# Lqm26/BMCNet-ESR

Hardware: AMD Instinct MI355X
Metric: LR-voxel-frames/sec x4 SR train step, NFS-shaped 180x240 (BASELINE configs[1] / [2]), f32 (higher is better)
Workload: dtype f32; 1 GPU; BMCNet(scale=4, n_c=128, n_b=5) x4 SR train step, NFS-shaped 180x240 (BASELINE configs[1] / [2]) -> 720x960, bs=4/GPU, arithmetic fp32 (native fp32 MFMA; 3x3 convolutions through Winograd F(4x4,3x3) / F(2x2,3x3) transforms in fp32), SEQL=9 SEQN=2 (8 windows BPTT), event scatter + fwd + MSE + bwd + Adam(amsgrad); global_batch=4, parallelism=dp1, rccl_ranks=1, rccl_initialised_before_headline_run=False

## Files before the change

### bmcnet-esr_amd/bmc_hip/lib.py

```python
from __future__ import annotations

import ctypes as C
import os

import torch

_HERE = os.path.dirname(os.path.abspath(__file__))
LIB_PATH = os.environ.get("BMC_HIP_LIB") or os.path.join(os.path.dirname(_HERE), "csrc", "libbmc_hip.so")

if not os.path.exists(LIB_PATH):
    raise ImportError(
        f"{LIB_PATH} not found: build the HIP extension first "
        "(python -c 'import __graft_entry__ as g; g.build()' or make -C bmcnet-esr_amd/csrc). "
        "The BMCNet MI355X path has no CPU fallback.")

_lib = C.CDLL(LIB_PATH)

MAX_SRC = 6
c_fp = C.c_void_p


class Src(C.Structure):
    _fields_ = [("ptr", C.c_void_p), ("batch_stride", C.c_longlong), ("pix_stride", C.c_int), ("nch", C.c_int),
                ("batch_shift", C.c_int), ("batch_mod", C.c_int)]


class ConvArgs(C.Structure):
    _fields_ = [("nsrc", C.c_int), ("src", Src * MAX_SRC), ("wpacked", C.c_void_p), ("bias", C.c_void_p),
                ("w_group_stride", C.c_longlong), ("bias_group_stride", C.c_int), ("batch_per_group", C.c_int),
                ("out", C.c_void_p), ("out_batch_stride", C.c_longlong), ("out_pix_stride", C.c_int),
                ("B", C.c_int), ("H", C.c_int), ("W", C.c_int), ("Cout", C.c_int), ("Coutpad", C.c_int),
                ("taps", C.c_int), ("relu", C.c_int), ("residual", Src), ("mask", Src), ("accumulate", C.c_int),
                ("math", C.c_int)]


class PgemmArgs(C.Structure):
    _fields_ = [("a", Src), ("nsrc", C.c_int), ("src", Src * MAX_SRC), ("B", C.c_int), ("H", C.c_int), ("W", C.c_int),
                ("taps", C.c_int), ("batch_per_group", C.c_int), ("slabs", C.c_void_p), ("nsplit", C.c_int),
                ("zeros", C.c_void_p), ("bias_slabs", C.c_void_p), ("math", C.c_int), ("tap_groups", C.c_int)]


class ChainFwdArgs(C.Structure):
    _fields_ = [("s0", Src), ("s1", Src), ("wstream", C.c_void_p), ("bias_f", C.c_void_p), ("bias_c", C.c_void_p),
                ("gamma", C.c_void_p), ("beta", C.c_void_p), ("eps", C.c_float), ("yhat", C.c_void_p), ("rstd", C.c_void_p),
                ("centre", C.c_void_p), ("B", C.c_int), ("C", C.c_int), ("H", C.c_int), ("W", C.c_int)]


class ChainBwdArgs(C.Structure):
    _fields_ = [("dcentre", Src), ("wstream", C.c_void_p), ("gamma", C.c_void_p), ("yhat", C.c_void_p), ("rstd", C.c_void_p),
                ("dz", C.c_void_p), ("ds1", C.c_void_p), ("ds0", C.c_void_p), ("ds0_add", Src), ("n", C.c_int), ("C", C.c_int),
                ("H", C.c_int), ("W", C.c_int)]


class MmTerm(C.Structure):
    _fields_ = [("a", C.c_void_p), ("a_sb", C.c_longlong), ("a_sg", C.c_longlong), ("a_si", C.c_int), ("a_sk", C.c_int),
                ("b", C.c_void_p), ("b_sb", C.c_longlong), ("b_sg", C.c_longlong), ("b_sk", C.c_int), ("b_sj", C.c_int),
                ("w", C.c_void_p), ("w_sb", C.c_longlong), ("w_sg", C.c_longlong), ("w_sk", C.c_int)]


class SmallMmArgs(C.Structure):
    _fields_ = [("nterms", C.c_int), ("t", MmTerm * 2), ("nbatch", C.c_int), ("batch_per_group", C.c_int),
                ("M", C.c_int), ("N", C.c_int), ("K", C.c_int), ("alpha", C.c_float),
                ("u", C.c_void_p), ("u_sb", C.c_longlong), ("u_sg", C.c_longlong),
                ("v", C.c_void_p), ("v_sb", C.c_longlong), ("v_sg", C.c_longlong),
                ("c", C.c_void_p), ("c_sb", C.c_longlong), ("c_sg", C.c_longlong), ("c_si", C.c_int), ("c_sj", C.c_int),
                ("vec_out", C.c_void_p), ("vo_sb", C.c_longlong), ("vo_sg", C.c_longlong), ("accumulate", C.c_int)]


def _sig(name, argtypes, restype=C.c_int):
    fn = getattr(_lib, name)
    fn.argtypes = argtypes
    fn.restype = restype
    return fn


_ll, _i, _f, _p = C.c_longlong, C.c_int, C.c_float, C.c_void_p

bmc_version = _sig("bmc_version", [])
bmc_last_error = _sig("bmc_last_error", [], C.c_char_p)
_events = _sig("bmc_events_to_channels", [_p, _p, _p, _p, _i, _i, _i, _p, _i, _p])
_voxel = _sig("bmc_events_to_voxel", [_p, _p, _p, _p, _p, _ll, _i, _i, _i, _i, _p, _i, _p, _p])
_stack_pol = _sig("bmc_events_to_stack_polarity", [_p, _p, _p, _p, _ll, _p, _p, _i, _i, _i, _p, _p, _i, _p])
_mask = _sig("bmc_events_to_mask", [_p, _p, _p, _ll, _i, _i, _p, _p, _i, _p])
_stack = _sig("bmc_events_to_stack", [_p, _p, _p, _p, _ll, _p, _p, _i, _i, _i, _p, _p, _i, _p])
_enc_raw = _sig("bmc_encode_raw_events", [_p, _p, _p, _p, _p, _i, _i, _i, _p, _p])
_events_ws = _sig("bmc_events_binned_ws_bytes", [_ll, _i, _i, _i], C.c_longlong)
_events_binned = _sig("bmc_events_to_channels_binned", [_p, _p, _p, _p, _ll, _i, _i, _i, _p, _i, _p, _ll, _p])
_enc_raw_binned = _sig("bmc_encode_raw_events_binned", [_p, _p, _p, _p, _p, _ll, _i, _i, _i, _p, _p, _ll, _p])
_ev_torch_ws = _sig("bmc_events_torch_ws_ints", [_ll, _i, _i], C.c_longlong)
_ev_img_torch = _sig("bmc_events_to_image_torch", [_p, _p, _p, _ll, _i, _i, _i, _i, _i, _p, _p, _p])
_ev_vox_torch = _sig("bmc_events_to_voxel_torch", [_p, _p, _p, _p, _ll, _i, _i, _i, _p, _p, _p])
_pack_w = _sig("bmc_pack_weight", [_p, _p, _i, _i, _i, _i, _i, _i, _p, _p])
_pack_wt = _sig("bmc_pack_weight_t", [_p, _p, _i, _i, _i, _i, _i, _i, _i, _i, _p, _p])
_pack_wino = _sig("bmc_pack_weight_wino", [_p, _p, _i, _i, _i, _i, _i, _i, _i, _i, _p, _p])
_pack_wino4 = _sig("bmc_pack_weight_wino4", [_p, _p, _i, _i, _i, _i, _i, _i, _i, _i, _p, _p])
_ww_nsplit = _sig("bmc_wgrad_wino_nsplit", [_i, _i, _i])
_stream_low = _sig("bmc_stream_create_low_priority", [C.POINTER(C.c_void_p)])
_small_mm = _sig("bmc_small_mm", [C.POINTER(SmallMmArgs), _p])
_ww = _sig("bmc_wgrad_wino", [C.POINTER(Src), C.POINTER(Src), _i, _i, _i, _i, _p, _p, _p])
_ww_red = _sig("bmc_wgrad_wino_reduce", [_p, _i, _p, _i, _i, _i, _p, _p, _p])
_ww_multi = _sig("bmc_wgrad_wino_multi", [C.POINTER(Src), C.POINTER(Src), C.POINTER(C.c_int), _i, _i, _i, _i, _p, _p, _p])
_ptr_table = _sig("bmc_ptr_table", [C.POINTER(C.c_ulonglong), _i, _p, _p])
_wino_rows = _sig("bmc_conv_wino_rows", [_i, _i, _i, _i, _i])
_ww4_nsplit = _sig("bmc_wgrad_wino4_nsplit", [_i, _i, _i])
_ww4 = _sig("bmc_wgrad_wino4", [C.POINTER(Src), C.POINTER(Src), _i, _i, _i, _i, _p, _p, _p])
_ww4_red = _sig("bmc_wgrad_wino4_reduce", [_p, _i, _p, _i, _i, _i, _p, _p, _p])
_split_w = _sig("bmc_split_weight", [_p, _p, _ll, _i, _i, _p])
_conv = _sig("bmc_conv", [C.POINTER(ConvArgs), _p])
_pgemm = _sig("bmc_pgemm", [C.POINTER(PgemmArgs), _p])
_red_w = _sig("bmc_pgemm_reduce_weight", [_p, _i, _i, _i, _i, _i, _p, _i, _p, _i, _p, _p, _p])
_red_wg = _sig("bmc_pgemm_reduce_weight_groups", [_p, _i, _i, _i, _i, _i, _p, _i, _p, _i, _p, _p, _p])
_red_p = _sig("bmc_pgemm_reduce_plain", [_p, _i, _i, _i, _i, _f, _p, _p])
_colsum = _sig("bmc_colsum", [_p, _ll, _i, _i, _p, _p, _i, _p])
_relu_bwd = _sig("bmc_relu_bwd", [_p, _p, _p, _ll, _p])
_ln_fwd = _sig("bmc_layernorm_fwd", [_p, _p, _p, _ll, _i, _f, _p, _p, _p])
_ln_bwd = _sig("bmc_layernorm_bwd", [_p, _p, _p, _p, _ll, _i, _p, _p, _p, _p, _i, _p])
_sm_fwd = _sig("bmc_softmax_fwd", [_p, _ll, _i, _p, _p])
_sm_bwd = _sig("bmc_softmax_bwd", [_p, _p, _ll, _i, _f, _p, _p])
_pack_in = _sig("bmc_pack_inputs", [_p, _ll, _ll, _ll, _ll, _ll, _i, _i, _i, _i, _p, _p, _p])
_unshuffle = _sig("bmc_unshuffle_to_nhwc", [_p, _i, _i, _i, _i, _i, _p, _i, _p])
_shuffle = _sig("bmc_shuffle_to_hr", [_p, _i, _i, _i, _i, _i, _p, _ll, _ll, _ll, _ll, _p, _i, _p])
_head_mse_fwd = _sig("bmc_head_mse_fwd", [_p, _i, _i, _i, _i, _i, _p, _ll, _ll, _ll, _ll, _p, _ll, _p, _p, _p, _p])
_head_mse_bwd = _sig("bmc_head_mse_bwd", [_p, _p, _p, _ll, _p, _i, _i, _i, _i, _i, _p, _p])
_group_sum = _sig("bmc_group_sum", [_p, _i, _ll, _p, _p])
_bicubic_fwd = _sig("bmc_bicubic_resize_fwd", [_p, _ll, _i, _i, _i, _i, _p, _p])
_bicubic_bwd = _sig("bmc_bicubic_resize_bwd", [_p, _ll, _i, _i, _i, _i, _p, _p])
_chain_fwd = _sig("bmc_chain_fwd", [C.POINTER(ChainFwdArgs), _p])
_chain_bwd = _sig("bmc_chain_bwd", [C.POINTER(ChainBwdArgs), _p])
_chain_affine = _sig("bmc_chain_affine_grads", [_p, _p, _p, _p, _p, _i, _p, _p, _p, _p, _i, _p])
_slot_stage = _sig("bmc_slot_stage", [_p, _i, _i, _i, _i, _p, _p, _i, _p, _i, _ll, _p, _ll, _p])
_slot_commit = _sig("bmc_slot_commit", [_p, _i, C.POINTER(C.c_void_p), _i, _ll, _p, _i, _p, _p, _ll, _p])
_slot_metrics = _sig("bmc_slot_metrics", [_p, _i, _p, _i, _i, _i, _i, _i, _i, _i, _p])
_slot_encode = _sig("bmc_slot_encode", [_p, _i, _i, _i, _i, _i, _i, _p, _p, _p])
_slot_emit = _sig("bmc_slot_emit", [_p, _p, _i, _p, _i, _i, _i, _i, _p, _p])
_slot_emit_timed = _sig("bmc_slot_emit_timed", [_p, _p, _i, _p, _i, _i, _i, _i, _p, _p, _p, _ll, _p])
_slot_emit_clocked = _sig("bmc_slot_emit_clocked", [_p, _p, _p, _i, _p, _i, _i, _i, _i, _p, _p, _p, _ll, _p])
_slot_emit_timed_ws = _sig("bmc_slot_emit_timed_scratch_bytes", [_i, _i, _ll], C.c_longlong)
_slot_hot_update = _sig("bmc_slot_hot_update", [_p, _p, _i, _i, _i, _i, _i, _i, _p, _p, _p, _p])
_slot_encode_filtered = _sig("bmc_slot_encode_filtered", [_p, _p, _p, _i, _i, _i, _i, _i, _i, _p, _p, _p])
_hot_pixel_mask = _sig("bmc_hot_pixel_mask", [_p, _i, _i, _i, _i, _f, _p, _p, _p])
_slot_render = _sig("bmc_slot_render", [_p, _p, _i, _i, _i, _i, _i, _p, _p])

EXPORTS = ["bmc_version", "bmc_last_error", "bmc_events_to_channels", "bmc_events_to_voxel", "bmc_events_to_stack", "bmc_encode_raw_events", "bmc_pack_weight", "bmc_pack_weight_t", "bmc_split_weight", "bmc_conv",
           "bmc_pgemm", "bmc_pgemm_reduce_weight", "bmc_pgemm_reduce_plain", "bmc_colsum", "bmc_relu_bwd",
           "bmc_layernorm_fwd", "bmc_layernorm_bwd", "bmc_softmax_fwd", "bmc_softmax_bwd", "bmc_pack_inputs",
           "bmc_unshuffle_to_nhwc", "bmc_shuffle_to_hr", "bmc_bicubic_resize_fwd", "bmc_bicubic_resize_bwd",
           "bmc_chain_fwd", "bmc_chain_bwd", "bmc_chain_affine_grads", "bmc_group_sum",
           "bmc_head_mse_fwd", "bmc_head_mse_bwd", "bmc_events_to_stack_polarity", "bmc_events_to_mask",
           "bmc_pgemm_reduce_weight_groups", "bmc_events_binned_ws_bytes", "bmc_events_to_channels_binned",
           "bmc_encode_raw_events_binned", "bmc_pack_weight_wino", "bmc_pack_weight_wino4", "bmc_wgrad_wino_nsplit", "bmc_wgrad_wino",
           "bmc_wgrad_wino_reduce", "bmc_events_torch_ws_ints", "bmc_events_to_image_torch",
           "bmc_events_to_voxel_torch", "bmc_stream_create_low_priority", "bmc_small_mm",
           "bmc_wgrad_wino4_nsplit", "bmc_wgrad_wino4", "bmc_wgrad_wino4_reduce", "bmc_wgrad_wino_multi", "bmc_ptr_table",
           "bmc_conv_wino_rows", "bmc_slot_stage", "bmc_slot_commit", "bmc_slot_metrics", "bmc_slot_encode", "bmc_slot_emit",
           "bmc_slot_emit_timed", "bmc_slot_emit_timed_scratch_bytes", "bmc_slot_emit_clocked", "bmc_slot_hot_update",
           "bmc_slot_encode_filtered", "bmc_hot_pixel_mask", "bmc_slot_render"]


def check(rc, what):
    if rc != 0:
        raise RuntimeError(f"{what} failed (rc={rc}): {bmc_last_error().decode()}")


def call(fn, what, *args):
    check(fn(*args), what)


def has_symbol(name: str) -> bool:
    return hasattr(_lib, name)
```

### bmcnet-esr_amd/csrc/pgemm.hip

```cpp
#include "bmc_common.h"
#include "pgemm_k.h"
#include "dma_ring.h"

namespace {


template <int TAPS, int TG = TAPS, bool TAB = false>
__global__ __launch_bounds__(512, 2) void pgemm_dma_kernel(const PgemmK a) {
    constexpr int HWD = PT_W + 2, HHT = PT_H + 2;
    constexpr int NHALO = TAPS == 9 ? HWD * HHT : PT;
    constexpr int XCH = TAPS == 9 ? 64 : 128;
    constexpr int NT = TAPS == 9 ? 1 : 2;
    constexpr int XSH = TAPS == 9 ? 4 : 5;
    constexpr int BUF = 2048 * 4;
    __shared__ __attribute__((aligned(16))) float lds[4 * BUF];
    __shared__ SrcDev tab[BMC_MAX_SRC];
    const int tid = threadIdx.x, lane = tid & 63;
    BMC_LOAD_SRC_TABLE(tab, a, tid);
    __syncthreads();
    const int wave = __builtin_amdgcn_readfirstlane(tid >> 6);
    const int li = lane & 31, lh = lane >> 5;
    const int mw = wave & 3, nw = wave >> 2;

    int bid = blockIdx.x;
    const int split = bid % a.nsplit; bid /= a.nsplit;
    const int tg = TG == TAPS ? 0 : bid % (TAPS / TG);
    if (TG != TAPS) bid /= TAPS / TG;
    const int nb = bid % a.n_nblk; bid /= a.n_nblk;
    const int mb = bid % a.n_mblk;
    const int g = bid / a.n_mblk;
    const int m0 = mb * 128, n0 = nb * XCH;
    const bool wave_active = m0 + 32 * mw < a.Mpad;
    const int HWp = a.H * a.W;

    f32x16 acc[TG * NT];
#pragma unroll
    for (int t = 0; t < TG * NT; ++t)
#pragma unroll
        for (int r = 0; r < 16; ++r) acc[t][r] = 0.f;

    const int ntiles = a.batch_per_group * a.tiles_per_img;
    int xsi = 0, xch0 = n0;
#pragma unroll
    for (int si = 1; si < BMC_MAX_SRC; ++si)
        if (xsi == si - 1 && xch0 >= tab[si - 1].nch && si < a.nsrc) { xch0 -= tab[si - 1].nch; xsi = si; }
    const SrcDev xs = tab[xsi];
    const bool x_one_src = xch0 + XCH <= xs.nch;
    int a_off[4], x_off[4], a_yx[4], x_yx[4];
#pragma unroll
    for (int i = 0; i < 4; ++i) {
        const int e = i * 512 + tid, p = e >> 5, c4 = (e & 31) * 4;
        a_yx[i] = TAPS == 9 ? ((p >> 4) << 16) | (p & 15) : p;
        a_off[i] = ((TAPS == 9 ? (p >> 4) * a.W + (p & 15) : p) * a.a.pix_stride + m0 + c4) * 4;
        const int hp = e >> XSH, xc4 = (e & ((1 << XSH) - 1)) * 4;
        const int hy = TAPS == 9 ? hp / HWD : 0, hx = TAPS == 9 ? hp - hy * HWD : hp;
        x_yx[i] = TAPS == 9 ? (hy << 16) | hx : hp;
        x_off[i] = ((TAPS == 9 ? (hp < NHALO ? hy * a.W + hx : 0) : hp) * xs.pix_stride + xch0 + xc4) * 4;
    }
    const bool all_ch = m0 + 128 <= a.M && n0 + XCH <= a.N && x_one_src &&
                        (long long)a.H * a.W * (a.a.pix_stride > xs.pix_stride ? a.a.pix_stride : xs.pix_stride) < (1ll << 28);
    const int step_img = a.nsplit / a.tiles_per_img, step_rem = a.nsplit - step_img * a.tiles_per_img;
    const int step_ty = TAPS == 9 ? step_rem / a.tiles_x : 0, step_tx = TAPS == 9 ? step_rem - step_ty * a.tiles_x : step_rem;
    int nx_bb = split / a.tiles_per_img, nx_ty, nx_tx;
    {
        const int tin = split - nx_bb * a.tiles_per_img;
        nx_ty = TAPS == 9 ? tin / a.tiles_x : 0; nx_tx = TAPS == 9 ? tin - nx_ty * a.tiles_x : tin;
    }
    auto dma = [&](const void* sbase, unsigned voff, float* ldst) { dma16(sbase, voff, lds_addr(ldst)); };
    auto issue = [&](int tile, int buf) {
        const int b = g * a.batch_per_group + nx_bb;
        int y0 = 0, x0 = 0, p0 = 0;
        if (TAPS == 9) { y0 = nx_ty * PT_H; x0 = nx_tx * PT_W; }
        else p0 = nx_tx * PT;
        nx_bb += step_img; nx_ty += step_ty; nx_tx += step_tx;
        if (TAPS == 9) {
            if (nx_tx >= a.tiles_x) { nx_tx -= a.tiles_x; ++nx_ty; }
            if (nx_ty >= a.tiles_y) { nx_ty -= a.tiles_y; ++nx_bb; }
        } else if (nx_tx >= a.tiles_per_img) { nx_tx -= a.tiles_per_img; ++nx_bb; }
        const float* ab = src_bp<TAB>(a.a, b);
        const bool interior = TAPS == 9 ? (y0 >= 1 && x0 >= 1 && y0 + PT_H + 1 <= a.H && x0 + PT_W + 1 <= a.W) : (p0 + PT <= HWp);
        if (interior && all_ch) {
            const float* const abt = ab + (TAPS == 9 ? (long long)y0 * a.W + x0 : (long long)p0) * a.a.pix_stride;
            const float* const xbt = src_bp<TAB>(xs, b) +
                                     (TAPS == 9 ? (long long)(y0 - 1) * a.W + (x0 - 1) : (long long)p0) * xs.pix_stride;
#pragma unroll
            for (int i = 0; i < 4; ++i) dma(abt, (unsigned)a_off[i], lds + buf * BUF + (i * 512 + wave * 64) * 4);
#pragma unroll
            for (int i = 0; i < 4; ++i) dma(xbt, (unsigned)x_off[i], lds + (2 + buf) * BUF + (i * 512 + wave * 64) * 4);
            return;
        }
#pragma unroll
        for (int i = 0; i < 4; ++i) {
            const int e = i * 512 + tid, p = e >> 5, c4 = (e & 31) * 4;
            long long pix;
            bool ok;
            if (TAPS == 9) {
                const int y = y0 + (p >> 4), x = x0 + (p & 15);
                ok = y < a.H && x < a.W;
                pix = (long long)y * a.W + x;
            } else {
                pix = p0 + p;
                ok = pix < HWp;
            }
            const float* src = a.zeros;
            if (ok && m0 + c4 < a.M) src = ab + pix * a.a.pix_stride + m0 + c4;
            dma16v(src, lds_addr(lds + buf * BUF + (i * 512 + wave * 64) * 4));
        }
#pragma unroll
        for (int i = 0; i < 4; ++i) {
            const int e = i * 512 + tid, hp = e >> XSH, c4 = (e & ((1 << XSH) - 1)) * 4;
            long long pix;
            bool ok;
            if (TAPS == 9) {
                const int hy = hp / HWD, hx = hp - hy * HWD;
                const int y = y0 - 1 + hy, x = x0 - 1 + hx;
                ok = hp < NHALO && y >= 0 && y < a.H && x >= 0 && x < a.W;
                pix = (long long)y * a.W + x;
            } else {
                pix = p0 + hp;
                ok = pix < HWp;
            }
            int ch = n0 + c4;
            const float* src = a.zeros;
            if (ok && ch < a.N) {
                int s_i = 0;
#pragma unroll
                for (int si = 1; si < BMC_MAX_SRC; ++si)
                    if (s_i == si - 1 && ch >= tab[si - 1].nch && si < a.nsrc) { ch -= tab[si - 1].nch; s_i = si; }
                const SrcDev S = tab[s_i];
                src = src_bp<TAB>(S, b) + pix * S.pix_stride + ch;
            }
            dma16v(src, lds_addr(lds + (2 + buf) * BUF + (i * 512 + wave * 64) * 4));
        }
    };

    if (split < ntiles) issue(split, 0);
    dma_wait<0>();
    __syncthreads();
    const bool do_bias = a.bias_slabs != nullptr && nb == 0 && tg == 0;
    float bsum = 0.f;
    int it = 0;
    for (int tile = split; tile < ntiles; tile += a.nsplit, ++it) {
        const int cur = it & 1;
        const int next = tile + a.nsplit;
        if (next < ntiles) issue(next, cur ^ 1);
        if (do_bias) {
            const float* const bp = lds + cur * BUF + (tid >> 7) * 16 * 128 + (tid & 127);
#pragma unroll
            for (int r = 0; r < 16; ++r) bsum += bp[r * 128];
        }
        if (wave_active) {
            const float* const ap = lds + cur * BUF + lh * 128 + 32 * mw + li;
            const float* const xp = lds + (2 + cur) * BUF + lh * XCH + 32 * NT * nw + li + (TG == TAPS ? 0 : tg * HWD * XCH);
            if constexpr (TAPS == 1) {
                constexpr int QB = 4, NBAT = PT / 2 / QB;
                float av[2][QB], xv[2][QB][NT];
                auto rd = [&](const int slot, const int q0) __attribute__((always_inline)) {
#pragma unroll
                    for (int j = 0; j < QB; ++j) {
                        av[slot][j] = ap[2 * (q0 + j) * 128];
#pragma unroll
                        for (int u = 0; u < NT; ++u) xv[slot][j][u] = xp[2 * (q0 + j) * XCH + 32 * u];
                    }
                };
                rd(0, 0);
#pragma unroll
                for (int qb = 0; qb < NBAT; ++qb) {
                    if (qb + 1 < NBAT) rd((qb + 1) & 1, (qb + 1) * QB);
                    __builtin_amdgcn_sched_barrier(0);
#pragma unroll
                    for (int j = 0; j < QB; ++j)
#pragma unroll
                        for (int u = 0; u < NT; ++u)
                            acc[u] = __builtin_amdgcn_mfma_f32_32x32x2f32(av[qb & 1][j], xv[qb & 1][j][u], acc[u], 0, 0, 0);
                    __builtin_amdgcn_sched_barrier(0);
                }
            } else
#pragma unroll
            for (int q = 0; q < PT / 2; ++q) {
                const float av = ap[2 * q * 128];
#pragma unroll
                for (int tap = 0; tap < TG; ++tap)
#pragma unroll
                    for (int u = 0; u < NT; ++u) {
                        int off;
                        if (TAPS == 9) off = (((q >> 3) + tap / 3) * HWD + 2 * (q & 7) + tap % 3) * XCH;
                        else off = 2 * q * XCH + 32 * u;
                        acc[tap * NT + u] = __builtin_amdgcn_mfma_f32_32x32x2f32(av, xp[off], acc[tap * NT + u], 0, 0, 0);
                    }
            }
        }
        dma_wait<0>();
        __syncthreads();
    }

    if (do_bias && m0 + (tid & 127) < a.Mpad)
        a.bias_slabs[(((long long)split * a.G + g) * 4 + (tid >> 7)) * a.Mpad + m0 + (tid & 127)] = bsum;
    if (wave_active) {
        float* const sl = a.slabs + (((long long)split * a.G + g) * TAPS + (TG == TAPS ? 0 : tg * TG)) * a.Mpad * a.Npad;
#pragma unroll
        for (int tap = 0; tap < TG; ++tap)
#pragma unroll
            for (int u = 0; u < NT; ++u) {
                const int n = n0 + 32 * NT * nw + 32 * u + li;
                if (n < a.Npad) {
#pragma unroll
                    for (int r = 0; r < 16; ++r) {
                        const int m = m0 + 32 * mw + (r & 3) + 8 * (r >> 2) + 4 * lh;
                        sl[((long long)tap * a.Mpad + m) * a.Npad + n] = acc[tap * NT + u][r];
                    }
                }
            }
    }
}

__device__ __forceinline__ float split_sum(const float* p, long long slab, int nsplit, float* red) {
    const int part = threadIdx.x >> 5, ol = threadIdx.x & 31;
    float s = 0.f;
    if (p)
        for (int i = part; i < nsplit; i += 8) s += p[i * slab];
    red[part * 32 + ol] = s;
    __syncthreads();
    float t = 0.f;
    if (part == 0) {
#pragma unroll
        for (int k = 0; k < 8; ++k) t += red[k * 32 + ol];
    }
    __syncthreads();
    return t;
}

struct GroupDst { float* dw[4]; float* db[4]; int n; };

constexpr int BIAS_OUT = 4;
__device__ __forceinline__ void bias_block_sum(const float* bias_slabs, int nsplit, int G, int M, int Mpad, float* db,
                                               int accumulate, int block, const GroupDst& gd, float* red ) {
    const long long total = (long long)G * M;
    const long long idx = (long long)block * BIAS_OUT + (threadIdx.x & (BIAS_OUT - 1));
    const bool live = idx < total;
    const int g = live ? (int)(idx / M) : 0, m = live ? (int)(idx % M) : 0;
    const int part = threadIdx.x / BIAS_OUT, nparts = 256 / BIAS_OUT, n4 = nsplit * 4;
    float s = 0.f;
    if (live) {
        auto at = [&](int i) { return ldg4(bias_slabs + (((long long)(i >> 2) * G + g) * 4 + (i & 3)) * Mpad + m); };
        int i = part;
        for (; i + 7 * nparts < n4; i += 8 * nparts) {
            float v[8];
#pragma unroll
            for (int k = 0; k < 8; ++k) v[k] = at(i + k * nparts);
#pragma unroll
            for (int k = 0; k < 8; ++k) s += v[k];
        }
        for (; i < n4; i += nparts) s += at(i);
    }
    red[threadIdx.x] = s;
    __syncthreads();
    if (threadIdx.x < BIAS_OUT && live) {
        float t = 0.f;
        for (int k = 0; k < nparts; ++k) t += red[k * BIAS_OUT + threadIdx.x];
        float* o = gd.n ? gd.db[g] + m : db + idx;
        *o = accumulate ? *o + t : t;
    }
}

__global__ void reduce_weight_kernel(const float* slabs, int nsplit, int G, int taps, int M, int N, int Mpad, int Npad,
                                     const int* kmap, int Cin, float* dw, int accumulate, const float* bias_slabs,
                                     float* db, int wblocks, const GroupDst gd) {
    __shared__ float red[256];
    if ((int)blockIdx.x >= wblocks) {
        bias_block_sum(bias_slabs, nsplit, G, M, Mpad, db, accumulate, (int)blockIdx.x - wblocks, gd, red);
        return;
    }
    const long long total = (long long)G * taps * M * N;
    const long long slab = (long long)G * taps * Mpad * Npad;
    const long long nchunk = (total + 31) / 32;
    for (long long chunk = blockIdx.x; chunk < nchunk; chunk += wblocks) {
        const long long idx = chunk * 32 + (threadIdx.x & 31);
        const float* p = nullptr;
        int m = 0, tap = 0, g = 0, ci = -1;
        if (idx < total) {
            const int n = idx % N;
            long long r = idx / N;
            m = r % M; r /= M;
            tap = r % taps;
            g = r / taps;
            ci = kmap ? kmap[n] : n;
            if (ci >= 0) p = slabs + (((long long)g * taps + tap) * Mpad + m) * Npad + n;
        }
        const float s = split_sum(p, slab, nsplit, red);
        if (threadIdx.x < 32 && ci >= 0) {
            float* o = (gd.n ? gd.dw[g] : dw + (long long)g * M * Cin * taps) + ((long long)m * Cin + ci) * taps + tap;
            *o = accumulate ? *o + s : s;
        }
    }
}

__global__ void reduce_weight4_kernel(const float* slabs, int nsplit, int G, int taps, int M, int N, int Mpad, int Npad,
                                      const int* kmap, int Cin, float* dw, int accumulate, const float* bias_slabs,
                                      float* db, int wblocks, const GroupDst gd, int P) {
    __shared__ f32x4 red4[256];
    __shared__ float red[256];
    if ((int)blockIdx.x >= wblocks) {
        bias_block_sum(bias_slabs, nsplit, G, M, Mpad, db, accumulate, (int)blockIdx.x - wblocks, gd, red);
        return;
    }
    const int per = 256 / P, ol = threadIdx.x % per, part = threadIdx.x / per;
    const int n4s = N / 4;
    const long long total4 = (long long)G * taps * M * n4s;
    const long long slab = (long long)G * taps * Mpad * Npad;
    const long long nchunk = (total4 + per - 1) / per;
    for (long long chunk = blockIdx.x; chunk < nchunk; chunk += wblocks) {
        const long long idx = chunk * per + ol;
        const bool live = idx < total4;
        int n = 0, m = 0, tap = 0, g = 0;
        if (live) {
            n = (int)(idx % n4s) * 4;
            long long r = idx / n4s;
            m = r % M; r /= M;
            tap = r % taps;
            g = r / taps;
        }
        f32x4 acc = {0.f, 0.f, 0.f, 0.f};
        float* o[4] = {nullptr, nullptr, nullptr, nullptr};
        float old[4] = {0.f, 0.f, 0.f, 0.f};
        if (live && part == 0) {
            float* const base = (gd.n ? gd.dw[g] : dw + (long long)g * M * Cin * taps) + (long long)m * Cin * taps + tap;
#pragma unroll
            for (int k = 0; k < 4; ++k) {
                const int ci = kmap ? kmap[n + k] : n + k;
                if (ci >= 0) {
                    o[k] = base + (long long)ci * taps;
                    if (accumulate) old[k] = ldg4(o[k]);
                }
            }
        }
        if (live) {
            const float* p = slabs + (((long long)g * taps + tap) * Mpad + m) * Npad + n;
            int i = part;
            for (; i + 3 * P < nsplit; i += 4 * P) {
                const f32x4 v0 = ldg16(p + (long long)i * slab), v1 = ldg16(p + (long long)(i + P) * slab);
                const f32x4 v2 = ldg16(p + (long long)(i + 2 * P) * slab), v3 = ldg16(p + (long long)(i + 3 * P) * slab);
                acc += v0; acc += v1; acc += v2; acc += v3;
            }
            for (; i < nsplit; i += P) acc += ldg16(p + (long long)i * slab);
        }
        if (P > 1) {
            red4[threadIdx.x] = acc;
            __syncthreads();
            if (part == 0) {
                acc = red4[ol];
                for (int k = 1; k < P; ++k) acc += red4[k * per + ol];
            }
            __syncthreads();
        }
#pragma unroll
        for (int k = 0; k < 4; ++k)
            if (o[k]) stg4(o[k], old[k] + acc[k]);
    }
}

__global__ void reduce_plain_kernel(const float* slabs, int nsplit, int G, int M, int N, int Mpad, int Npad, float scale,
                                    float* out) {
    __shared__ float red[256];
    const long long total = (long long)G * M * N;
    const long long slab = (long long)G * Mpad * Npad;
    const long long nchunk = (total + 31) / 32;
    for (long long chunk = blockIdx.x; chunk < nchunk; chunk += gridDim.x) {
        const long long idx = chunk * 32 + (threadIdx.x & 31);
        const float* p = nullptr;
        if (idx < total) {
            const int n = idx % N;
            long long r = idx / N;
            const int m = r % M;
            const int g = r / M;
            p = slabs + ((long long)g * Mpad + m) * Npad + n;
        }
        const float s = split_sum(p, slab, nsplit, red);
        if (threadIdx.x < 32 && idx < total) out[idx] = s * scale;
    }
}

}

extern "C" int bmc_pgemm(const bmc_pgemm_args_t* h, bmc_stream_t stream) {
    BMC_CHECK_ARG(h != nullptr, "bmc_pgemm: null args");
    BMC_CHECK_ARG(h->nsrc >= 1 && h->nsrc <= BMC_MAX_SRC, "bmc_pgemm: nsrc=%d out of range", h->nsrc);
    BMC_CHECK_ARG(h->taps == 1 || h->taps == 9, "bmc_pgemm: taps must be 1 or 9");
    BMC_CHECK_ARG(h->tap_groups == 0 || h->tap_groups == 1 || (h->tap_groups == 3 && h->taps == 9 && h->math != BMC_MATH_BF16X6),
                  "bmc_pgemm: tap_groups must be 0, 1, or 3 (3: taps = 9, fp32 or bf16 arithmetic)");
    BMC_CHECK_ARG(h->batch_per_group >= 1 && h->B % h->batch_per_group == 0, "bmc_pgemm: B %% batch_per_group != 0");
    BMC_CHECK_ARG(h->nsplit >= 1 && h->slabs, "bmc_pgemm: nsplit/slabs");
    BMC_CHECK_ARG(h->zeros != nullptr, "bmc_pgemm: the zero buffer is required");
    BMC_CHECK_ARG(h->a.ptr && h->a.nch > 0 && h->a.nch % 4 == 0 && h->a.pix_stride % 4 == 0, "bmc_pgemm: bad A operand");
    PgemmK k;
    k.a = to_dev(h->a);
    k.nsrc = h->nsrc;
    int N = 0;
    for (int i = 0; i < BMC_MAX_SRC; ++i) {
        if (i < h->nsrc) {
            BMC_CHECK_ARG(h->src[i].ptr && h->src[i].nch > 0 && h->src[i].nch % 4 == 0 && h->src[i].pix_stride % 4 == 0,
                          "bmc_pgemm: bad source %d", i);
            k.src[i] = to_dev(h->src[i]);
            N += h->src[i].nch;
        } else k.src[i] = to_dev(h->src[0]);
    }
    k.B = h->B; k.H = h->H; k.W = h->W; k.batch_per_group = h->batch_per_group;
    k.slabs = h->slabs; k.nsplit = h->nsplit; k.zeros = h->zeros; k.bias_slabs = h->bias_slabs;
    k.M = h->a.nch; k.Mpad = bmc_round_up(k.M, 32); k.N = N; k.Npad = bmc_round_up(N, 32);
    k.G = h->B / h->batch_per_group;
    k.tap_groups = h->tap_groups == 3 ? 3 : 1;
    k.n_mblk = (k.Mpad + 127) / 128;
    hipStream_t st = (hipStream_t)stream;
    BMC_CHECK_ARG(h->math == BMC_MATH_FP32 || h->math == BMC_MATH_BF16 || h->math == BMC_MATH_BF16X6,
                  "bmc_pgemm: unknown math mode %d", h->math);
    if (h->math != BMC_MATH_FP32) {
        const int cols = bmc_pgemm_cols(h->taps, h->math);
        k.n_nblk = (k.Npad + cols - 1) / cols;
        if (h->taps == 9) {
            k.tiles_x = (h->W + PT_W - 1) / PT_W; k.tiles_y = (h->H + PT_H - 1) / PT_H;
            k.tiles_per_img = k.tiles_x * k.tiles_y;
        } else {
            k.tiles_x = k.tiles_y = 0;
            k.tiles_per_img = (h->H * h->W + PT - 1) / PT;
        }
        return bmc_pgemm_bf_launch(k, h->taps, h->math == BMC_MATH_BF16 ? 1 : 3, st);
    }
    const bool tab = pgemm_uses_tables(k);
    if (h->taps == 9) {
        k.n_nblk = (k.Npad + 63) / 64;
        k.tiles_x = (h->W + PT_W - 1) / PT_W; k.tiles_y = (h->H + PT_H - 1) / PT_H;
        k.tiles_per_img = k.tiles_x * k.tiles_y;
        if (h->tap_groups == 3) {
            dim3 grid((unsigned)((long long)k.G * k.n_mblk * k.n_nblk * 3 * k.nsplit));
            if (tab) hipLaunchKernelGGL((pgemm_dma_kernel<9, 3, true>), grid, dim3(512), 0, st, k);
            else hipLaunchKernelGGL((pgemm_dma_kernel<9, 3>), grid, dim3(512), 0, st, k);
        } else {
            dim3 grid((unsigned)((long long)k.G * k.n_mblk * k.n_nblk * k.nsplit));
            if (tab) hipLaunchKernelGGL((pgemm_dma_kernel<9, 9, true>), grid, dim3(512), 0, st, k);
            else hipLaunchKernelGGL(pgemm_dma_kernel<9>, grid, dim3(512), 0, st, k);
        }
    } else {
        k.n_nblk = (k.Npad + 127) / 128;
        k.tiles_x = k.tiles_y = 0;
        k.tiles_per_img = (h->H * h->W + PT - 1) / PT;
        dim3 grid((unsigned)((long long)k.G * k.n_mblk * k.n_nblk * k.nsplit));
        if (tab) hipLaunchKernelGGL((pgemm_dma_kernel<1, 1, true>), grid, dim3(512), 0, st, k);
        else hipLaunchKernelGGL(pgemm_dma_kernel<1>, grid, dim3(512), 0, st, k);
    }
    BMC_CHECK_LAUNCH("bmc_pgemm");
    return 0;
}

static int reduce_parts(int nsplit) { return nsplit <= 4 ? 1 : nsplit <= 8 ? 2 : nsplit <= 16 ? 4 : nsplit <= 64 ? 8 : nsplit <= 128 ? 16 : 32; }

extern "C" int bmc_pgemm_reduce_weight(const float* slabs, int nsplit, int G, int taps, int M, int N, const int* kmap,
                                       int Cin, float* dw, int accumulate, const float* bias_slabs, float* db,
                                       bmc_stream_t stream) {
    BMC_CHECK_ARG(slabs && dw && nsplit >= 1, "bmc_pgemm_reduce_weight: bad args");
    BMC_CHECK_ARG((bias_slabs == nullptr) == (db == nullptr), "bmc_pgemm_reduce_weight: bias_slabs and db go together");
    const long long total = (long long)G * taps * M * N;
    const int wblocks = (int)((total + 31) / 32 > 8192 ? 8192 : (total + 31) / 32);
    const int bblocks = bias_slabs ? (int)(((long long)G * M + BIAS_OUT - 1) / BIAS_OUT) : 0;
    GroupDst gd = {};
    if (N % 4 == 0) {
        const int P = reduce_parts(nsplit), per = 256 / P;
        const long long nchunk = ((long long)G * taps * M * (N / 4) + per - 1) / per;
        const int wb4 = (int)(nchunk > 8192 ? 8192 : nchunk);
        hipLaunchKernelGGL(reduce_weight4_kernel, dim3(wb4 + bblocks), dim3(256), 0, (hipStream_t)stream, slabs, nsplit, G, taps,
                           M, N, bmc_round_up(M, 32), bmc_round_up(N, 32), kmap, Cin, dw, accumulate, bias_slabs, db, wb4, gd, P);
    } else
        hipLaunchKernelGGL(reduce_weight_kernel, dim3(wblocks + bblocks), dim3(256), 0, (hipStream_t)stream, slabs, nsplit, G,
                           taps, M, N, bmc_round_up(M, 32), bmc_round_up(N, 32), kmap, Cin, dw, accumulate, bias_slabs, db,
                           wblocks, gd);
    BMC_CHECK_LAUNCH("bmc_pgemm_reduce_weight");
    return 0;
}

extern "C" int bmc_pgemm_reduce_weight_groups(const float* slabs, int nsplit, int G, int taps, int M, int N, const int* kmap,
                                              int Cin, float* const* dw, int accumulate, const float* bias_slabs,
                                              float* const* db, bmc_stream_t stream) {
    BMC_CHECK_ARG(slabs && dw && nsplit >= 1 && G >= 1 && G <= 4, "bmc_pgemm_reduce_weight_groups: bad args (1 <= G <= 4)");
    BMC_CHECK_ARG((bias_slabs == nullptr) == (db == nullptr), "bmc_pgemm_reduce_weight_groups: bias_slabs and db go together");
    GroupDst gd = {};
    gd.n = G;
    for (int g = 0; g < G; ++g) {
        BMC_CHECK_ARG(dw[g] && (!db || db[g]), "bmc_pgemm_reduce_weight_groups: null destination for group %d", g);
        gd.dw[g] = dw[g];
        gd.db[g] = db ? db[g] : nullptr;
    }
    const long long total = (long long)G * taps * M * N;
    const int wblocks = (int)((total + 31) / 32 > 8192 ? 8192 : (total + 31) / 32);
    const int bblocks = bias_slabs ? (int)(((long long)G * M + BIAS_OUT - 1) / BIAS_OUT) : 0;
    if (N % 4 == 0) {
        const int P = reduce_parts(nsplit), per = 256 / P;
        const long long nchunk = ((long long)G * taps * M * (N / 4) + per - 1) / per;
        const int wb4 = (int)(nchunk > 8192 ? 8192 : nchunk);
        hipLaunchKernelGGL(reduce_weight4_kernel, dim3(wb4 + bblocks), dim3(256), 0, (hipStream_t)stream, slabs, nsplit, G, taps,
                           M, N, bmc_round_up(M, 32), bmc_round_up(N, 32), kmap, Cin, nullptr, accumulate, bias_slabs, nullptr,
                           wb4, gd, P);
    } else
        hipLaunchKernelGGL(reduce_weight_kernel, dim3(wblocks + bblocks), dim3(256), 0, (hipStream_t)stream, slabs, nsplit, G,
                           taps, M, N, bmc_round_up(M, 32), bmc_round_up(N, 32), kmap, Cin, nullptr, accumulate, bias_slabs,
                           nullptr, wblocks, gd);
    BMC_CHECK_LAUNCH("bmc_pgemm_reduce_weight_groups");
    return 0;
}

extern "C" int bmc_pgemm_reduce_plain(const float* slabs, int nsplit, int G, int M, int N, float scale, float* out,
                                      bmc_stream_t stream) {
    BMC_CHECK_ARG(slabs && out && nsplit >= 1, "bmc_pgemm_reduce_plain: bad args");
    const long long total = (long long)G * M * N;
    const int blocks = (int)((total + 31) / 32 > 8192 ? 8192 : (total + 31) / 32);
    hipLaunchKernelGGL(reduce_plain_kernel, dim3(blocks), dim3(256), 0, (hipStream_t)stream, slabs, nsplit, G, M, N,
                       bmc_round_up(M, 32), bmc_round_up(N, 32), scale, out);
    BMC_CHECK_LAUNCH("bmc_pgemm_reduce_plain");
    return 0;
}
```

### include/bmc_hip.h

```cpp
#ifndef BMC_HIP_H
#define BMC_HIP_H

#ifdef __cplusplus
extern "C" {
#endif

typedef void* bmc_stream_t;

#define BMC_MAX_SRC 6
#define BMC_CK 16

typedef struct bmc_src {
    const float* ptr;
    long long batch_stride;
    int pix_stride;
    int nch;
    int batch_shift;
    int batch_mod;
} bmc_src_t;
#define BMC_SRC_TABLE (-1)


int bmc_version(void);
const char* bmc_last_error(void);
int bmc_stream_create_low_priority(bmc_stream_t* out);

int bmc_events_to_channels(float* xs, float* ys, const float* ps, const long long* offsets,
                           int nframes, int H, int W, float* out, int mutate, bmc_stream_t s);

long long bmc_events_binned_ws_bytes(long long nevents, int nframes, int H, int W);
int bmc_events_to_channels_binned(float* xs, float* ys, const float* ps, const long long* offsets, long long nevents,
                                  int nframes, int H, int W, float* out, int mutate, void* ws, long long ws_bytes,
                                  bmc_stream_t s);
int bmc_encode_raw_events_binned(const short* xs, const short* ys, const double* ps, const long long* offsets,
                                 const unsigned char* flips, long long nevents, int nframes, int H, int W, float* out,
                                 void* ws, long long ws_bytes, bmc_stream_t s);

long long bmc_events_torch_ws_ints(long long n, int H, int W);
int bmc_events_to_image_torch(float* xs, float* ys, float* ps, long long n, int H, int W, int clip_out_of_range, int bilinear,
                              int padding, float* out, int* ws, bmc_stream_t s);
int bmc_events_to_voxel_torch(float* xs, float* ys, const float* ts, const float* ps, long long n, int bins, int H, int W,
                              float* out, int* ws, bmc_stream_t s);

int bmc_events_to_voxel(float* xs, float* ys, const float* ts, const float* ps, const long long* offsets,
                        long long nevents, int nframes, int bins, int H, int W, float* out, int mutate, int* ws,
                        bmc_stream_t s);

int bmc_events_to_stack(float* xs, float* ys, const float* ts, float* ps, long long n, const float* tstart,
                        const float* tend, int bins, int H, int W, float* out, int* ranges, int mutate, bmc_stream_t s);

int bmc_events_to_stack_polarity(float* xs, float* ys, const float* ts, const float* ps, long long n, const float* tstart,
                                 const float* tend, int bins, int H, int W, float* out, int* ranges, int mutate,
                                 bmc_stream_t s);

int bmc_events_to_mask(float* xs, float* ys, float* ps, long long n, int H, int W, float* out, int* ws, int mutate,
                       bmc_stream_t s);

int bmc_encode_raw_events(const short* xs, const short* ys, const double* ps, const long long* offsets,
                          const unsigned char* flips, int nframes, int H, int W, float* out, bmc_stream_t s);

int bmc_pack_weight(const float* w, const int* kmap, int G, int Cout, int Cin, int taps,
                    int Kpad, int Coutpad, float* out, bmc_stream_t s);
int bmc_pack_weight_t(const float* w, const int* kmap, int G, int Cout, int Cin, int taps,
                      int k0, int nk, int nkpad, int Coutpad16, float* out, bmc_stream_t s);
#define BMC_MATH_FP32 0
#define BMC_MATH_BF16 1
#define BMC_MATH_BF16X6 3
#define BMC_MATH_FP32_WINO 4
#define BMC_MATH_FP32_WINO4 5
int bmc_split_weight(const float* packed, void* out, long long nsteps, int Coutpad, int planes, bmc_stream_t s);

int bmc_pack_weight_wino(const float* w, const int* kmap, int G, int Cout, int Cin, int Kpad, int Coutpad, int transposed,
                         int k0, int nk, float* out, bmc_stream_t s);

int bmc_conv_wino_rows(int B, int H, int W, int Coutpad, int cus);

int bmc_pack_weight_wino4(const float* w, const int* kmap, int G, int Cout, int Cin, int Kpad, int Coutpad, int transposed,
                          int k0, int nk, float* out, bmc_stream_t s);

typedef struct bmc_conv_args {
    int nsrc;
    bmc_src_t src[BMC_MAX_SRC];
    const void* wpacked;
    const float* bias;
    long long w_group_stride;
    int bias_group_stride;
    int batch_per_group;
    float* out;
    long long out_batch_stride;
    int out_pix_stride;
    int B, H, W;
    int Cout, Coutpad;
    int taps;
    int relu;
    bmc_src_t residual;
    bmc_src_t mask;
    int accumulate;
    int math;
} bmc_conv_args_t;
int bmc_conv(const bmc_conv_args_t* host_args, bmc_stream_t s);

typedef struct bmc_pgemm_args {
    bmc_src_t a;
    int nsrc;
    bmc_src_t src[BMC_MAX_SRC];
    int B, H, W, taps;
    int batch_per_group;
    float* slabs;
    int nsplit;
    const float* zeros;
    float* bias_slabs;
    int math;
    int tap_groups;
} bmc_pgemm_args_t;
int bmc_pgemm(const bmc_pgemm_args_t* host_args, bmc_stream_t s);
int bmc_pgemm_reduce_weight(const float* slabs, int nsplit, int G, int taps, int M, int N, const int* kmap,
                            int Cin, float* dw, int accumulate, const float* bias_slabs ,
                            float* db , bmc_stream_t s);
int bmc_pgemm_reduce_weight_groups(const float* slabs, int nsplit, int G, int taps, int M, int N, const int* kmap,
                                   int Cin, float* const* dw, int accumulate, const float* bias_slabs, float* const* db,
                                   bmc_stream_t s);
int bmc_pgemm_reduce_plain(const float* slabs, int nsplit, int G, int M, int N, float scale,
                           float* out, bmc_stream_t s);

int bmc_wgrad_wino_nsplit(int B, int H, int W);
int bmc_wgrad_wino(const bmc_src_t* dy, const bmc_src_t* x, int B, int H, int W, int nsplit, float* part, float* bias_part,
                   bmc_stream_t s);
int bmc_wgrad_wino_reduce(const float* part, int nsplit, float* dw, int ldw, int k0, int accumulate, const float* bias_part,
                          float* db, bmc_stream_t s);
int bmc_wgrad_wino_multi(const bmc_src_t* dy, const bmc_src_t* x, const int* batches, int nseg, int H, int W, int nsplit,
                         float* part, float* bias_part, bmc_stream_t s);

int bmc_wgrad_wino4_nsplit(int B, int H, int W);
int bmc_wgrad_wino4(const bmc_src_t* dy, const bmc_src_t* x, int B, int H, int W, int nsplit, float* part, float* bias_part,
                    bmc_stream_t s);
int bmc_wgrad_wino4_reduce(const float* part, int nsplit, float* dw, int ldw, int k0, int accumulate, const float* bias_part,
                           float* db, bmc_stream_t s);

int bmc_ptr_table(const unsigned long long* ptrs, int n, unsigned long long* table, bmc_stream_t s);

int bmc_group_sum(const float* in, int groups, long long n, float* out, bmc_stream_t s);
int bmc_colsum(const float* x, long long npix, int pix_stride, int C, float* ws, float* out,
               int accumulate, bmc_stream_t s);
int bmc_relu_bwd(const float* dy, const float* y, float* g, long long n, bmc_stream_t s);
int bmc_layernorm_fwd(const float* x, const float* gamma, const float* beta, long long npix, int C,
                      float eps, float* y, float* stats, bmc_stream_t s);
int bmc_layernorm_bwd(const float* dy, const float* x, const float* stats, const float* gamma,
                      long long npix, int C, float* dx, float* ws, float* dgamma, float* dbeta,
                      int accumulate, bmc_stream_t s);
int bmc_softmax_fwd(const float* a, long long rows, int C, float* p, bmc_stream_t s);
int bmc_softmax_bwd(const float* p, const float* dp, long long rows, int C, float scale_out,
                    float* da, bmc_stream_t s);

int bmc_pack_inputs(const float* x, long long sb, long long sc, long long st, long long sy, long long sx,
                    int B, int H, int W, int repeat, float* xin_p, float* xin_n, bmc_stream_t s);
int bmc_unshuffle_to_nhwc(const float* hr, int B, int C, int H, int W, int r, float* lr, int split, bmc_stream_t s);
int bmc_shuffle_to_hr(const float* lr, int B, int C, int H, int W, int r, const float* base,
                      long long sb, long long sc, long long sy, long long sx, float* hr, int split ,
                      bmc_stream_t s);

int bmc_head_mse_fwd(const float* lr, int B, int C, int H, int W, int r, const float* base, long long sb, long long sc,
                     long long sy, long long sx, const float* gt, long long gt_batch_stride, float* hr, float* partials,
                     float* loss, bmc_stream_t s);
int bmc_head_mse_bwd(const float* dpred, const float* pred, const float* gt, long long gt_batch_stride, const float* gloss,
                     int B, int C, int H, int W, int r, float* dlr, bmc_stream_t s);

typedef struct bmc_chain_fwd_args {
    bmc_src_t s0, s1;
    const float* wstream;
    const float* bias_f;
    const float* bias_c;
    const float* gamma;
    const float* beta;
    float eps;
    float* yhat;
    float* rstd;
    float* centre;
    int B, C, H, W;
} bmc_chain_fwd_args_t;
int bmc_chain_fwd(const bmc_chain_fwd_args_t* host_args, bmc_stream_t s);

typedef struct bmc_chain_bwd_args {
    bmc_src_t dcentre;
    const float* wstream;
    const float* gamma;
    const float* yhat;
    const float* rstd;
    float* dz;
    float* ds1;
    float* ds0;
    bmc_src_t ds0_add;
    int n, C, H, W;
} bmc_chain_bwd_args_t;
int bmc_chain_bwd(const bmc_chain_bwd_args_t* host_args, bmc_stream_t s);
int bmc_chain_affine_grads(const float* G, const float* dbc, const float* Wc, const float* gamma, const float* beta, int C,
                           float* dwc, float* dbc_out, float* dgamma, float* dbeta, int accumulate, bmc_stream_t s);

typedef struct {
    const float* a; long long a_sb, a_sg; int a_si, a_sk;
    const float* b; long long b_sb, b_sg; int b_sk, b_sj;
    const float* w; long long w_sb, w_sg; int w_sk;
} bmc_mm_term_t;
typedef struct {
    int nterms;
    bmc_mm_term_t t[2];
    int nbatch, batch_per_group;
    int M, N, K;
    float alpha;
    const float* u; long long u_sb, u_sg;
    const float* v; long long v_sb, v_sg;
    float* c; long long c_sb, c_sg; int c_si, c_sj;
    float* vec_out; long long vo_sb, vo_sg;
    int accumulate;
} bmc_small_mm_args_t;
int bmc_small_mm(const bmc_small_mm_args_t* host_args, bmc_stream_t s);

int bmc_bicubic_resize_fwd(const float* x, long long planes, int H, int W, int Ho, int Wo, float* y, bmc_stream_t s);
int bmc_bicubic_resize_bwd(const float* gy, long long planes, int H, int W, int Ho, int Wo, float* gx, bmc_stream_t s);

#define BMC_MAX_SLOTS 256
#define BMC_SLOT_ACTIVE 1
#define BMC_SLOT_RESET 2
typedef struct bmc_slot {
    const float* frames;
    const float* gt;
    float* keep;
    double* result;
    int flags;
    int pad_;
} bmc_slot_t;

int bmc_slot_stage(const bmc_slot_t* table, int S, int seqn, int H, int W, float* x, const void* feat_pool, int pool_bf16,
                   float* feat, int nfeat, long long feat_n, float* pred, long long pred_n, bmc_stream_t s);
int bmc_slot_commit(const bmc_slot_t* table, int S, const float* const* feat_src, int nfeat, long long feat_n, void* feat_pool,
                    int pool_bf16, const float* pred_src, float* pred_pool, long long pred_n, bmc_stream_t s);
#define BMC_SLOT_MAX_PARTS 64
int bmc_slot_metrics(const bmc_slot_t* table, int S, const float* pred, int sH, int sW, int H, int W, int gh, int gw,
                     int nparts, bmc_stream_t s);

#define BMC_SLOT_MAX_SEQN 8
typedef struct bmc_slot_events {
    const short* lr_xs;
    const short* lr_ys;
    const double* lr_ps;
    const short* gt_xs;
    const short* gt_ys;
    const double* gt_ps;
    long long gt_range[2];
    long long lr_range[BMC_SLOT_MAX_SEQN][2];
} bmc_slot_events_t;
int bmc_slot_encode(const bmc_slot_events_t* table, int S, int seqn, int H, int W, int gh, int gw, float* lr_scratch,
                    float* gt_scratch, bmc_stream_t s);

typedef struct bmc_slot_emit {
    short* xs;
    short* ys;
    signed char* ps;
    const long long* index_in;
    long long* index_out;
    long long capacity;
} bmc_slot_emit_t;
#define BMC_SLOT_EMIT_MAX_PARTS 1024
int bmc_slot_emit(const bmc_slot_t* table, const bmc_slot_emit_t* emit, int S, const float* pred, int sH, int sW, int max_count,
                  int nparts, unsigned* parts, bmc_stream_t s);

#define BMC_EVENT_T0 0.01
#define BMC_EVENT_T1 1.0
#define BMC_SLOT_EMIT_TIMED_MAX_COUNT 255
#define BMC_SLOT_EMIT_TIMED_BLOCK 4096
#define BMC_SLOT_EMIT_TIMED_MAX_WINDOW (1ll << 28)
typedef struct bmc_slot_emit_timed {
    short* xs;
    short* ys;
    signed char* ps;
    const long long* index_in;
    long long* index_out;
    long long capacity;
    float* ts;
} bmc_slot_emit_timed_t;
long long bmc_slot_emit_timed_scratch_bytes(int S, int nparts, long long window_capacity);
int bmc_slot_emit_timed(const bmc_slot_t* table, const bmc_slot_emit_timed_t* emit, int S, const float* pred, int sH, int sW,
                        int max_count, int nparts, unsigned* parts, const unsigned short* rank_table, void* scratch,
                        long long window_capacity, bmc_stream_t s);

typedef struct bmc_slot_clock {
    double t_first;
    double t_last;
    double* ts;
} bmc_slot_clock_t;
int bmc_slot_emit_clocked(const bmc_slot_t* table, const bmc_slot_emit_timed_t* emit, const bmc_slot_clock_t* clock, int S,
                          const float* pred, int sH, int sW, int max_count, int nparts, unsigned* parts,
                          const unsigned short* rank_table, void* scratch, long long window_capacity, bmc_stream_t s);

typedef struct bmc_slot_hot {
    int* hot_pixels;
    unsigned char* hot_mask;
    int first_item;
    int new_from;
    int active;
    int pad_;
    int cmin[BMC_SLOT_MAX_SEQN];
} bmc_slot_hot_t;
int bmc_slot_hot_update(const bmc_slot_hot_t* hot, const bmc_slot_events_t* events, int S, int seqn, int H, int W, int max_px,
                        int negative_rate, int* counts, unsigned char* ring, int* ws, bmc_stream_t s);
int bmc_slot_encode_filtered(const bmc_slot_events_t* table, const bmc_slot_hot_t* hot, const unsigned char* ring, int S, int seqn,
                             int H, int W, int gh, int gw, float* lr_scratch, float* gt_scratch, bmc_stream_t s);
int bmc_hot_pixel_mask(float* event_rate, int H, int W, int active, int max_px, float max_rate, float* mask, unsigned* ws,
                       bmc_stream_t s);

#define BMC_SLOT_RENDER_MAX_PIXELS (1 << 24)
#define BMC_SLOT_RENDER_MAX_PARTS 1024
typedef struct bmc_slot_render {
    const float* src;
    unsigned char* dst;
} bmc_slot_render_t;
int bmc_slot_render(const bmc_slot_t* table, const bmc_slot_render_t* render, int S, int h, int w, int round, int nparts,
                    float* scratch, bmc_stream_t s);

#ifdef __cplusplus
}
#endif
#endif
```

Before: 47.12 LR-voxel-frames/s.

## Split K across idle waves in all-taps 3x3 pgemm for narrow M or N

When the padded M or N of the all-taps 3x3 weight-gradient pgemm is only 32 wide, most of the 8 waves in a block were inactive. The change reassigns those waves to separate slices of the pixel (K) dimension, then reduces the partial accumulators through LDS before the wave with ks==0 writes the slabs. This uses idle MFMA capacity on small-channel layers. The cost is an extra LDS reduction pass with barriers, and possible register or LDS pressure.

Result: faster. 47.73 LR-voxel-frames/s (median of 6 runs) (+1.3%).

```diff
diff --git a/bmcnet-esr_amd/bmc_hip/lib.py b/bmcnet-esr_amd/bmc_hip/lib.py
--- a/bmcnet-esr_amd/bmc_hip/lib.py
+++ b/bmcnet-esr_amd/bmc_hip/lib.py
@@ -108,6 +108,7 @@
 _split_w = _sig("bmc_split_weight", [_p, _p, _ll, _i, _i, _p])
 _conv = _sig("bmc_conv", [C.POINTER(ConvArgs), _p])
 _pgemm = _sig("bmc_pgemm", [C.POINTER(PgemmArgs), _p])
+pgemm_wave_map = _sig("bmc_pgemm_wave_map", [_i, _i, _i])
 _red_w = _sig("bmc_pgemm_reduce_weight", [_p, _i, _i, _i, _i, _i, _p, _i, _p, _i, _p, _p, _p])
 _red_wg = _sig("bmc_pgemm_reduce_weight_groups", [_p, _i, _i, _i, _i, _i, _p, _i, _p, _i, _p, _p, _p])
 _red_p = _sig("bmc_pgemm_reduce_plain", [_p, _i, _i, _i, _i, _f, _p, _p])
@@ -142,7 +143,7 @@
 _slot_render = _sig("bmc_slot_render", [_p, _p, _i, _i, _i, _i, _i, _p, _p])
 
 EXPORTS = ["bmc_version", "bmc_last_error", "bmc_events_to_channels", "bmc_events_to_voxel", "bmc_events_to_stack", "bmc_encode_raw_events", "bmc_pack_weight", "bmc_pack_weight_t", "bmc_split_weight", "bmc_conv",
-           "bmc_pgemm", "bmc_pgemm_reduce_weight", "bmc_pgemm_reduce_plain", "bmc_colsum", "bmc_relu_bwd",
+           "bmc_pgemm", "bmc_pgemm_wave_map", "bmc_pgemm_reduce_weight", "bmc_pgemm_reduce_plain", "bmc_colsum", "bmc_relu_bwd",
            "bmc_layernorm_fwd", "bmc_layernorm_bwd", "bmc_softmax_fwd", "bmc_softmax_bwd", "bmc_pack_inputs",
            "bmc_unshuffle_to_nhwc", "bmc_shuffle_to_hr", "bmc_bicubic_resize_fwd", "bmc_bicubic_resize_bwd",
            "bmc_chain_fwd", "bmc_chain_bwd", "bmc_chain_affine_grads", "bmc_group_sum",
diff --git a/bmcnet-esr_amd/csrc/pgemm.hip b/bmcnet-esr_amd/csrc/pgemm.hip
--- a/bmcnet-esr_amd/csrc/pgemm.hip
+++ b/bmcnet-esr_amd/csrc/pgemm.hip
@@ -5,8 +5,9 @@
 namespace {
 
 
-template <int TAPS, int TG = TAPS, bool TAB = false>
+template <int TAPS, int TG = TAPS, bool TAB = false, int KS = 1>
 __global__ __launch_bounds__(512, 2) void pgemm_dma_kernel(const PgemmK a) {
+    static_assert(KS == 1 || ((KS == 2 || KS == 4) && TAPS == 9 && TG == 9), "k-step shares: the all-taps 3x3 kernel only");
     constexpr int HWD = PT_W + 2, HHT = PT_H + 2;
     constexpr int NHALO = TAPS == 9 ? HWD * HHT : PT;
     constexpr int XCH = TAPS == 9 ? 64 : 128;
@@ -20,7 +21,8 @@
     __syncthreads();
     const int wave = __builtin_amdgcn_readfirstlane(tid >> 6);
     const int li = lane & 31, lh = lane >> 5;
-    const int mw = wave & 3, nw = wave >> 2;
+    const int mw = KS == 4 ? 0 : wave & 3, nw = KS == 1 ? wave >> 2 : KS == 2 ? 0 : wave & 1;
+    const int ks = KS == 1 ? 0 : KS == 2 ? wave >> 2 : wave >> 1;
 
     int bid = blockIdx.x;
     const int split = bid % a.nsplit; bid /= a.nsplit;
@@ -30,7 +32,7 @@
     const int mb = bid % a.n_mblk;
     const int g = bid / a.n_mblk;
     const int m0 = mb * 128, n0 = nb * XCH;
-    const bool wave_active = m0 + 32 * mw < a.Mpad;
+    const bool wave_active = KS == 4 ? n0 + 32 * nw < a.Npad : m0 + 32 * mw < a.Mpad;
     const int HWp = a.H * a.W;
 
     f32x16 acc[TG * NT];
@@ -150,8 +152,9 @@
             for (int r = 0; r < 16; ++r) bsum += bp[r * 128];
         }
         if (wave_active) {
-            const float* const ap = lds + cur * BUF + lh * 128 + 32 * mw + li;
-            const float* const xp = lds + (2 + cur) * BUF + lh * XCH + 32 * NT * nw + li + (TG == TAPS ? 0 : tg * HWD * XCH);
+            const float* const ap = lds + cur * BUF + lh * 128 + 32 * mw + li + (KS == 1 ? 0 : ks * (PT / KS) * 128);
+            const float* const xp = lds + (2 + cur) * BUF + lh * XCH + 32 * NT * nw + li + (TG == TAPS ? 0 : tg * HWD * XCH) +
+                                    (KS == 1 ? 0 : ks * (PT_H / KS) * HWD * XCH);
             if constexpr (TAPS == 1) {
                 constexpr int QB = 4, NBAT = PT / 2 / QB;
                 float av[2][QB], xv[2][QB][NT];
@@ -177,7 +180,7 @@
                 }
             } else
 #pragma unroll
-            for (int q = 0; q < PT / 2; ++q) {
+            for (int q = 0; q < PT / 2 / KS; ++q) {
                 const float av = ap[2 * q * 128];
 #pragma unroll
                 for (int tap = 0; tap < TG; ++tap)
@@ -196,7 +199,33 @@
 
     if (do_bias && m0 + (tid & 127) < a.Mpad)
         a.bias_slabs[(((long long)split * a.G + g) * 4 + (tid >> 7)) * a.Mpad + m0 + (tid & 127)] = bsum;
-    if (wave_active) {
+    if constexpr (KS > 1) {
+        constexpr int NG = 8 / KS, PASS = 3 * 16 * 64;
+        const int grp = KS == 2 ? mw : nw;
+#pragma unroll
+        for (int t0 = 0; t0 < TG; t0 += 3) {
+            if (ks > 0 && wave_active) {
+                float* const w = lds + ((ks - 1) * NG + grp) * PASS + lane;
+#pragma unroll
+                for (int t = 0; t < 3; ++t)
+#pragma unroll
+                    for (int r = 0; r < 16; ++r) w[(t * 16 + r) * 64] = acc[t0 + t][r];
+            }
+            __syncthreads();
+            if (ks == 0 && wave_active) {
+#pragma unroll 1
+                for (int k = 1; k < KS; ++k) {
+                    const float* const rd = lds + ((k - 1) * NG + grp) * PASS + lane;
+#pragma unroll
+                    for (int t = 0; t < 3; ++t)
+#pragma unroll
+                        for (int r = 0; r < 16; ++r) acc[t0 + t][r] += rd[(t * 16 + r) * 64];
+                }
+            }
+            __syncthreads();
+        }
+    }
+    if (wave_active && ks == 0) {
         float* const sl = a.slabs + (((long long)split * a.G + g) * TAPS + (TG == TAPS ? 0 : tg * TG)) * a.Mpad * a.Npad;
 #pragma unroll
         for (int tap = 0; tap < TG; ++tap)
@@ -380,6 +409,16 @@
     }
 }
 
+}
+
+static int pgemm_wave_map(int taps, int Mpad, int Npad) {
+    if (taps != 9) return 1;
+    if (Mpad <= 32) return 4;
+    return Npad <= 32 ? 2 : 1;
+}
+
+extern "C" int bmc_pgemm_wave_map(int taps, int M, int N) {
+    return pgemm_wave_map(taps, bmc_round_up(M, 32), bmc_round_up(N, 32));
 }
 
 extern "C" int bmc_pgemm(const bmc_pgemm_args_t* h, bmc_stream_t stream) {
@@ -436,7 +475,14 @@
             else hipLaunchKernelGGL((pgemm_dma_kernel<9, 3>), grid, dim3(512), 0, st, k);
         } else {
             dim3 grid((unsigned)((long long)k.G * k.n_mblk * k.n_nblk * k.nsplit));
-            if (tab) hipLaunchKernelGGL((pgemm_dma_kernel<9, 9, true>), grid, dim3(512), 0, st, k);
+            const int ksh = pgemm_wave_map(9, k.Mpad, k.Npad);
+            if (ksh == 2) {
+                if (tab) hipLaunchKernelGGL((pgemm_dma_kernel<9, 9, true, 2>), grid, dim3(512), 0, st, k);
+                else hipLaunchKernelGGL((pgemm_dma_kernel<9, 9, false, 2>), grid, dim3(512), 0, st, k);
+            } else if (ksh == 4) {
+                if (tab) hipLaunchKernelGGL((pgemm_dma_kernel<9, 9, true, 4>), grid, dim3(512), 0, st, k);
+                else hipLaunchKernelGGL((pgemm_dma_kernel<9, 9, false, 4>), grid, dim3(512), 0, st, k);
+            } else if (tab) hipLaunchKernelGGL((pgemm_dma_kernel<9, 9, true>), grid, dim3(512), 0, st, k);
             else hipLaunchKernelGGL(pgemm_dma_kernel<9>, grid, dim3(512), 0, st, k);
         }
     } else {
diff --git a/include/bmc_hip.h b/include/bmc_hip.h
--- a/include/bmc_hip.h
+++ b/include/bmc_hip.h
@@ -114,6 +114,7 @@
     int tap_groups;
 } bmc_pgemm_args_t;
 int bmc_pgemm(const bmc_pgemm_args_t* host_args, bmc_stream_t s);
+int bmc_pgemm_wave_map(int taps, int M, int N);
 int bmc_pgemm_reduce_weight(const float* slabs, int nsplit, int G, int taps, int M, int N, const int* kmap,
                             int Cin, float* dw, int accumulate, const float* bias_slabs ,
                             float* db , bmc_stream_t s);
```
